# xipengwang/AprilSAM

Hardware: NVIDIA H100
Metric: Gauss-Newton solves/sec (batch + incremental) on M3500 & 100k-pose graph (higher is better)
Workload: dtype f64

## Files before the change

aprilsam_b200/csrc/asam_cuda.cu:

```cuda

#include <cuda_runtime.h>

#include <cmath>
#include <cstdarg>
#include <cstdint>
#include <cstdio>
#include <cstdlib>
#include <cstring>
#include <ctime>

#include "asam_cuda.h"

#define ASAM_EXPORT extern "C" __attribute__((visibility("default")))

static thread_local char g_err[512] = "";

static int set_err(const char *fmt, ...)
{
    va_list ap;
    va_start(ap, fmt);
    vsnprintf(g_err, sizeof(g_err), fmt, ap);
    va_end(ap);
    return 1;
}
// ... 457 lines not shown
        return set_err("no CUDA device");
    int dev = 0;
    const char *e = getenv("ASAM_DEVICE");
    if (!e)
        e = getenv("LOCAL_RANK");
    if (e)
        dev = atoi(e) % n;
    CK(cudaSetDevice(dev));
    asam_dev *d = new asam_dev();
    d->device = dev;
    cudaDeviceProp prop;
    CK(cudaGetDeviceProperties(&prop, dev));
    d->n_sm = prop.multiProcessorCount;
    CK(cudaStreamCreateWithFlags(&d->stream, cudaStreamNonBlocking));
    d->pin_cap = 8u << 20;
    CK(cudaMallocHost((void **) &d->pin, d->pin_cap));
    CK(cudaMalloc((void **) &d->dstage, d->pin_cap));
    d->items = (BatchItem *) malloc(ASAM_TABLE_BYTES);
    CK(cudaEventCreateWithFlags(&d->up_ev, cudaEventDisableTiming));
    d->pin_down_cap = 8u << 20;
    CK(cudaMallocHost((void **) &d->pin_down, d->pin_down_cap));
    for (int i = 0; i < 6; i++)
        CK(cudaEventCreate(&d->ev[i]));
    if (buf_reserve(d, d->ctrl, 8 * sizeof(int), false, true))
        return 1;

    int max_optin = 0;
    CK(cudaDeviceGetAttribute(&max_optin, cudaDevAttrMaxSharedMemoryPerBlockOptin, dev));
    const int want = 200 * 1024;
    if (want > max_optin - 1024)
        return set_err("k_factor needs %d KB of shared memory per block, the device offers %d KB", want / 1024,
                       (max_optin - 1024) / 1024);
    d->fac_smem = want;
    CK(cudaFuncSetAttribute(k_factor, cudaFuncAttributeMaxDynamicSharedMemorySize, d->fac_smem));
    int occ = 0;
    CK(cudaOccupancyMaxActiveBlocksPerMultiprocessor(&occ, k_factor, d->fac_threads, d->fac_smem));
    if (occ < 1)
        return set_err("k_factor does not fit on an SM");
    d->fac_grid = occ * d->n_sm;

    d->leaf_smem = ASAM_LEAF_WARPS * ASAM_LEAF_STRIDE * (int) sizeof(double);
    CK(cudaFuncSetAttribute(k_factor_leaf, cudaFuncAttributeMaxDynamicSharedMemorySize, d->leaf_smem));
    CK(cudaOccupancyMaxActiveBlocksPerMultiprocessor(&occ, k_factor_leaf, 32 * ASAM_LEAF_WARPS, d->leaf_smem));
    if (occ < 1)
        return set_err("k_factor_leaf does not fit on an SM");
    d->leaf_grid = occ * d->n_sm;

    d->bsl_smem = ASAM_BSL_WARPS * ASAM_BSL_STRIDE * (int) sizeof(double);
    CK(cudaFuncSetAttribute(k_backsolve_leaf, cudaFuncAttributeMaxDynamicSharedMemorySize, d->bsl_smem));
    CK(cudaOccupancyMaxActiveBlocksPerMultiprocessor(&occ, k_backsolve_leaf, 32 * ASAM_BSL_WARPS, d->bsl_smem));
    if (occ < 1)
        return set_err("k_backsolve_leaf does not fit on an SM");
    d->bsl_grid = occ * d->n_sm;

    if (getenv("ASAM_BS_THREADS"))
        d->bs_threads = atoi(getenv("ASAM_BS_THREADS")) >= 256 ? 256 : 128;
    d->bs_smem = 100 * 1024;
    CK(cudaFuncSetAttribute(k_backsolve, cudaFuncAttributeMaxDynamicSharedMemorySize, d->bs_smem));
    CK(cudaOccupancyMaxActiveBlocksPerMultiprocessor(&occ, k_backsolve, d->bs_threads, d->bs_smem));
    if (occ < 1)
        return set_err("k_backsolve does not fit on an SM");
    d->bs_grid = occ * d->n_sm;
    CK(cudaFuncSetAttribute(k_step, cudaFuncAttributeMaxDynamicSharedMemorySize, d->fac_smem));
    if (getenv("ASAM_SOLO_PB") && atoi(getenv("ASAM_SOLO_PB")) >= 12)
        d->solo_pb = atoi(getenv("ASAM_SOLO_PB")) / 12 * 12;
    if (getenv("ASAM_PB_SMEM") && atoi(getenv("ASAM_PB_SMEM")) >= 3)
        d->pb_smem = atoi(getenv("ASAM_PB_SMEM")) / 3 * 3;
    if (getenv("ASAM_SMEM_MMA"))
        d->smem_mma = atoi(getenv("ASAM_SMEM_MMA"));
    if (getenv("ASAM_DIAG_MMA")) {
        const int v = atoi(getenv("ASAM_DIAG_MMA")) != 0;
        CK(cudaMemcpyToSymbol(g_diag_mma, &v, sizeof(int)));
    }
    if (getenv("ASAM_DMAP_AHEAD")) {
        const int v = atoi(getenv("ASAM_DMAP_AHEAD")) != 0;
        CK(cudaMemcpyToSymbol(g_dmap_ahead, &v, sizeof(int)));
    }
    if (getenv("ASAM_PF_GROUPS")) {
        const int v = atoi(getenv("ASAM_PF_GROUPS")) != 0;
        CK(cudaMemcpyToSymbol(g_pf_groups, &v, sizeof(int)));
    }
    if (getenv("ASAM_KEEP"))
        d->keep_off = atoi(getenv("ASAM_KEEP")) == 0;
    if (getenv("ASAM_TILE_MODE"))
        d->tile_mode = atoi(getenv("ASAM_TILE_MODE"));
    if (getenv("ASAM_SMALL_STEP"))
        d->small_ok = atoi(getenv("ASAM_SMALL_STEP")) != 0;
    memset(d->pin_down, 0, 64);
    *out = d;
    return 0;
}

ASAM_EXPORT void asam_dev_destroy(asam_dev_t *d)
{
    if (!d)
        return;
    cudaSetDevice(d->device);
    cudaStreamSynchronize(d->stream);
    Buf *all[] = { &d->f_type, &d->f_a, &d->f_b, &d->f_z, &d->f_W, &d->f_slot, &d->lp, &d->st, &d->node2q, &d->q2node,
                   &d->Adiag, &d->Aoff, &d->Bq, &d->y, &d->x, &d->dinv, &d->sn, &d->ipool, &d->arena, &d->arrive,
                   &d->xdone, &d->xblk, &d->tbar, &d->tasks_full, &d->nwait_full, &d->btasks_full, &d->tasks_tmp, &d->nwait_tmp,
                   &d->btasks_tmp, &d->keep_tmp, &d->leaf_tasks, &d->top_tasks, &d->top_nwait, &d->ctrl, &d->partial, &d->patch_ids, &d->patch_desc, &d->pts, &d->flush, &d->trace_fac, &d->trace_bs, &d->ptrace };
    for (int i = 0; i < 2; i++)
        if (d->tev[i])
            cudaEventDestroy(d->tev[i]);
    for (Buf *b : all)
        if (b->p)
            cudaFree(b->p);
    if (d->pin)
        cudaFreeHost(d->pin);
    if (d->pin_down)
        cudaFreeHost(d->pin_down);
    if (d->dstage)
        cudaFree(d->dstage);
    if (d->up_ev)
        cudaEventDestroy(d->up_ev);
    free(d->items);
    free(d->pend);
    free(d->sh_owner); free(d->sh_q0); free(d->sh_qn); free(d->sh_off); free(d->sh_cnt);
    for (int i = 0; i < 6; i++)
        if (d->ev[i])
            cudaEventDestroy(d->ev[i]);
    cudaStreamDestroy(d->stream);
    delete d;
}

ASAM_EXPORT int asam_reserve(asam_dev_t *d, int n_nodes, int n_factors, int n_slots, int n_sn, int64_t ipool_ints,
                             int64_t arena_doubles)
{
    CK(cudaSetDevice(d->device));
    size_t N = (size_t) (n_nodes > 0 ? n_nodes : 0), Fn = (size_t) (n_factors > 0 ? n_factors : 0);
    size_t S = (size_t) (n_slots > 0 ? n_slots : 0), SN = (size_t) (n_sn > 0 ? n_sn : 0);
    int rc = 0;
    rc |= buf_reserve(d, d->f_type, Fn * sizeof(int), true, false);
    rc |= buf_reserve(d, d->f_a, Fn * sizeof(int), true, false);
    rc |= buf_reserve(d, d->f_b, Fn * sizeof(int), true, false);
    rc |= buf_reserve(d, d->f_slot, Fn * sizeof(int), true, false);
    rc |= buf_reserve(d, d->f_z, Fn * 3 * sizeof(double), true, false);
    rc |= buf_reserve(d, d->f_W, Fn * 9 * sizeof(double), true, false);
    rc |= buf_reserve(d, d->lp, N * 3 * sizeof(double), true, false);
    rc |= buf_reserve(d, d->st, N * 3 * sizeof(double), true, false);
    rc |= buf_reserve(d, d->node2q, N * sizeof(int), true, false);
    rc |= buf_reserve(d, d->q2node, N * sizeof(int), true, false);
    rc |= buf_reserve(d, d->Adiag, N * 9 * sizeof(double), true, true);
    rc |= buf_reserve(d, d->Bq, N * 3 * sizeof(double), true, true);
    rc |= buf_reserve(d, d->y, N * 3 * sizeof(double), true, true);
    rc |= buf_reserve(d, d->x, N * 3 * sizeof(double), true, true);
    rc |= buf_reserve(d, d->dinv, N * 3 * sizeof(double), true, true);
    rc |= buf_reserve(d, d->Aoff, S * 9 * sizeof(double), true, true);
    rc |= buf_reserve(d, d->sn, SN * sizeof(asam_sn_desc_t), true, false);
    rc |= buf_reserve(d, d->arrive, SN * sizeof(int), true, true);
    rc |= buf_reserve(d, d->xdone, SN * sizeof(int), true, true);
    rc |= buf_reserve(d, d->xblk, SN * sizeof(int), true, true);
    rc |= buf_reserve(d, d->tbar, 2 * SN * sizeof(int), true, true);
    rc |= buf_reserve(d, d->ipool, (size_t) ipool_ints * sizeof(int), true, false);
    rc |= buf_reserve(d, d->arena, (size_t) arena_doubles * sizeof(double), true, false);
    return rc;
}

ASAM_EXPORT int asam_upload_factors(asam_dev_t *d, int first, int count, const int32_t *type, const int32_t *na,
                                    const int32_t *nb, const double *z3, const double *W9)
{
    if (count <= 0)
        return 0;
    size_t need = (size_t) first + count;
    if (need * sizeof(int) > d->f_type.cap)
        return set_err("asam_upload_factors: capacity (call asam_reserve)");
    int rc = 0;
    rc |= upload(d, (int *) d->f_type.p + first, type, count * sizeof(int));
    rc |= upload(d, (int *) d->f_a.p + first, na, count * sizeof(int));
    rc |= upload(d, (int *) d->f_b.p + first, nb, count * sizeof(int));
    rc |= upload(d, (double *) d->f_z.p + 3 * (size_t) first, z3, count * 3 * sizeof(double));
    rc |= upload(d, (double *) d->f_W.p + 9 * (size_t) first, W9, count * 9 * sizeof(double));
    return rc;
}

ASAM_EXPORT int asam_upload_points(asam_dev_t *d, int which, int first, int count, const double *p3)
{
    if (count <= 0)
        return 0;
    Buf &b = which == 0 ? d->lp : d->st;
    if (((size_t) first + count) * 3 * sizeof(double) > b.cap)
        return set_err("asam_upload_points: capacity");
    return upload(d, (double *) b.p + 3 * (size_t) first, p3, (size_t) count * 3 * sizeof(double));
}

ASAM_EXPORT int asam_copy_points(asam_dev_t *d, int from, int to, int first, int count)
{
    if (count <= 0 || from == to)
        return 0;
    CK(cudaSetDevice(d->device));
    Buf &src = from == 0 ? d->lp : d->st, &dst = to == 0 ? d->lp : d->st;
    const size_t off = (size_t) first * 3 * sizeof(double), bytes = (size_t) count * 3 * sizeof(double);
    if (off + bytes > src.cap || off + bytes > dst.cap)
        return set_err("asam_copy_points: capacity");
    if (flush_uploads(d))
        return 1;
    CK(cudaMemcpyAsync((char *) dst.p + off, (const char *) src.p + off, bytes, cudaMemcpyDeviceToDevice, d->stream));
    return 0;
}

ASAM_EXPORT int asam_upload_node2q(asam_dev_t *d, int first, int count, const int32_t *node2q)
{
    if (count <= 0)
        return 0;
    if (((size_t) first + count) * sizeof(int) > d->node2q.cap)
        return set_err("asam_upload_node2q: capacity");
    return upload(d, (int *) d->node2q.p + first, node2q, (size_t) count * sizeof(int));
}

ASAM_EXPORT int asam_upload_q2node(asam_dev_t *d, int first, int count, const int32_t *q2node)
{
    if (count <= 0)
        return 0;
    if (((size_t) first + count) * sizeof(int) > d->q2node.cap)
        return set_err("asam_upload_q2node: capacity");
    return upload(d, (int *) d->q2node.p + first, q2node, (size_t) count * sizeof(int));
}

ASAM_EXPORT int asam_upload_fslot(asam_dev_t *d, int first, int count, const int32_t *fslot)
{
    if (count <= 0)
        return 0;
    if (((size_t) first + count) * sizeof(int) > d->f_slot.cap)
        return set_err("asam_upload_fslot: capacity");
    return upload(d, (int *) d->f_slot.p + first, fslot, (size_t) count * sizeof(int));
}

ASAM_EXPORT int asam_upload_ipool(asam_dev_t *d, int64_t first, int64_t count, const int32_t *data)
{
    if (count <= 0)
        return 0;
    if ((size_t) (first + count) * sizeof(int) > d->ipool.cap)
        return set_err("asam_upload_ipool: capacity");
    return upload(d, (int *) d->ipool.p + first, data, (size_t) count * sizeof(int));
}

ASAM_EXPORT int asam_upload_desc(asam_dev_t *d, int n, const int32_t *sn_ids, const asam_sn_desc_t *desc)
{
    if (n <= 0)
        return 0;
    CK(cudaSetDevice(d->device));
    if (n <= 256) {
        for (int i = 0; i < n; i++)
            if (upload(d, (asam_sn_desc_t *) d->sn.p + sn_ids[i], &desc[i], sizeof(asam_sn_desc_t)))
                return 1;
        return 0;
    }
    if (buf_reserve(d, d->patch_ids, (size_t) n * sizeof(int), false, false))
        return 1;
    if (buf_reserve(d, d->patch_desc, (size_t) n * sizeof(asam_sn_desc_t), false, false))
        return 1;
    if (upload(d, d->patch_ids.p, sn_ids, (size_t) n * sizeof(int)))
        return 1;
    if (upload(d, d->patch_desc.p, desc, (size_t) n * sizeof(asam_sn_desc_t)))
        return 1;
    if (flush_uploads(d))
        return 1;
    k_apply_desc<<<(n + 127) / 128, 128, 0, d->stream>>>((asam_sn_desc_t *) d->sn.p, (const int *) d->patch_ids.p,
                                                         (const asam_sn_desc_t *) d->patch_desc.p, n);
    d->n_launch++;
    CK(cudaGetLastError());
    return 0;
}

ASAM_EXPORT int asam_hessian_reset(asam_dev_t *d, int n_nodes, int n_slots, int n_lambda, double lambda)
{
    CK(cudaSetDevice(d->device));
    size_t total = 9 * (size_t) n_nodes + 9 * (size_t) n_slots + 3 * (size_t) n_nodes;
    if (total == 0)
        return 0;
    if (flush_uploads(d))
        return 1;
    k_hessian_reset<<<(unsigned) ((total + 255) / 256), 256, 0, d->stream>>>(
        (double *) d->Adiag.p, (double *) d->Aoff.p, (double *) d->Bq.p, n_nodes, n_slots, n_lambda, lambda);
    d->n_launch++;
    CK(cudaGetLastError());
    return 0;
}

ASAM_EXPORT int asam_hessian_clear_range(asam_dev_t *d, int q_first, int q_count, int slot_first, int slot_count)
{
    CK(cudaSetDevice(d->device));
    int rc = 0;
    if (q_count > 0) {
        rc |= queue_fill(d, (double *) d->Adiag.p + 9 * (size_t) q_first, 0, (size_t) q_count * 9 * sizeof(double));
        rc |= queue_fill(d, (double *) d->Bq.p + 3 * (size_t) q_first, 0, (size_t) q_count * 3 * sizeof(double));
    }
    if (slot_count > 0)
        rc |= queue_fill(d, (double *) d->Aoff.p + 9 * (size_t) slot_first, 0, (size_t) slot_count * 9 * sizeof(double));
    return rc;
}

ASAM_EXPORT int asam_linearize(asam_dev_t *d, int f_first, int f_count, const double *pts6)
{
    if (f_count <= 0)
        return 0;
    CK(cudaSetDevice(d->device));
    LinArgs a;
    a.f_type = (const int *) d->f_type.p;
    a.f_a = (const int *) d->f_a.p;
    a.f_b = (const int *) d->f_b.p;
    a.f_slot = (const int *) d->f_slot.p;
    a.f_z = (const double *) d->f_z.p;
    a.f_W = (const double *) d->f_W.p;
    a.lp = (const double *) d->lp.p;
    a.st = (const double *) d->st.p;
// ... 759 lines not shown
```

aprilsam_b200/csrc/asam_kernels.cuh:

```cuda
#pragma once

#include <cuda_runtime.h>

#include <cstdint>

#include "asam_cuda.h"

#define ASAM_TR_FLAG (1 << 30)
#define ASAM_MAX_CACHED_CHILDREN 24

__device__ __forceinline__ double d_mod2pi(double v)
{
    const double twopi = 6.2831853071795862319959;
    const double pi = 3.141592653589793238462643383279502884196;
    double w = v + pi;
    return (w - twopi * floor(w / twopi)) - pi;
}

__device__ __forceinline__ void d_atb(const double *A, const double *B, double *C)
{
#pragma unroll
    for (int i = 0; i < 3; i++)
#pragma unroll
        for (int j = 0; j < 3; j++) {
// ... 554 lines not shown
                    for (int u = 0; u < 8; u++)
                        Li[lane + 32 * u + pp * ASAM_LDI] = vi[h][u];
                }
            }
        }
    }
    const int g = lane >> 2, t = lane & 3;
    const int r0 = warp * 8 * MT;
    const int nnt = (ncol + 7) >> 3;
    const int rowmax = rb0 + min(r0 + 8 * MT, nrow) - 1;
    const int nneed = (r0 < nrow && rowmax >= cb0) ? min(nnt, ((rowmax - cb0) >> 3) + 1) : 0;
    double acc[MT][8][2];
#pragma unroll
    for (int mt = 0; mt < MT; mt++)
#pragma unroll
        for (int q = 0; q < 8; q++)
#pragma unroll
            for (int e = 0; e < 2; e++) {
                const int ii = r0 + 8 * mt + g, jj = 8 * q + 2 * t + e;
                const bool ok = q < nneed && ii < nrow && jj < ncol && rb0 + ii >= cb0 + jj;
                acc[mt][q][e] = ok ? __ldcg(&F[(rb0 + ii) + (size_t) (cb0 + jj) * ld]) : 0.0;
            }
    if (bulk) {
        mbar_wait(bar, parity);
        parity ^= 1u;
    }
    __syncthreads();
    if (nneed > 0) {
        const double *ai = Li + shi + r0 + g + (size_t) t * ASAM_LDI;
        const double *bj_ = Lj + shj + g + (size_t) t * ASAM_LDJ;
#pragma unroll 2
        for (int kk = 0; kk < pb4; kk += 4) {
            double av[MT];
#pragma unroll
            for (int mt = 0; mt < MT; mt++)
                av[mt] = -ai[8 * mt + (size_t) kk * ASAM_LDI];
#pragma unroll
            for (int q = 0; q < 8; q++) {
                if (q < nneed) {
                    const double bv = bj_[8 * q + (size_t) kk * ASAM_LDJ];
#pragma unroll
                    for (int mt = 0; mt < MT; mt++)
                        dmma_8x8x4(acc[mt][q][0], acc[mt][q][1], av[mt], bv);
                }
            }
        }
#pragma unroll
        for (int mt = 0; mt < MT; mt++)
#pragma unroll
            for (int q = 0; q < 8; q++)
#pragma unroll
                for (int e = 0; e < 2; e++) {
                    const int ii = r0 + 8 * mt + g, jj = 8 * q + 2 * t + e;
                    if (q < nneed && ii < nrow && jj < ncol && rb0 + ii >= cb0 + jj) {
                        F[(rb0 + ii) + (size_t) (cb0 + jj) * ld] = acc[mt][q][e];
                        if (Dout)
                            Dout[ii + jj * ASAM_TPB] = acc[mt][q][e];
                    }
                }
    }
}

#define ASAM_LDW 52
#define ASAM_WS_DOUBLES(m) (2 * (size_t) ((m) + 2) * ASAM_LDW)

template <int MT>
__device__ __noinline__ void tile_rm(double *F, const int ld, const double *Wk, const int pb4, const int cb0, const int ncol,
                                     const int rb0, const int nrow, const int out_mode, double *Out, double *Li, double *Lj,
                                     unsigned long long *bar, unsigned &parity)
{
    const int tid = threadIdx.x;
    const int lane = tid & 31, warp = tid >> 5;
    const bool same = rb0 == cb0 && nrow >= ncol;
    __syncthreads();
    if (warp == 0) {
        asm volatile("fence.proxy.async;" ::: "memory");
        if (lane == 0) {
            const unsigned bi = (unsigned) nrow * ASAM_LDW * 8u, bj = same ? 0u : (unsigned) ncol * ASAM_LDW * 8u;
            mbar_expect_tx(bar, bi + bj);
            bulk_g2s(Li, Wk + (size_t) rb0 * ASAM_LDW, bi, bar);
            if (!same)
                bulk_g2s(Lj, Wk + (size_t) cb0 * ASAM_LDW, bj, bar);
        }
    }
    const double *Ljs = same ? Li : Lj;
    const int g = lane >> 2, t = lane & 3;
    const int r0 = warp * 8 * MT;
    const int nnt = (ncol + 7) >> 3;
    const int rowmax = rb0 + min(r0 + 8 * MT, nrow) - 1;
    const int nneed = (r0 < nrow && rowmax >= cb0) ? min(nnt, ((rowmax - cb0) >> 3) + 1) : 0;
    double acc[MT][8][2];
#pragma unroll
    for (int mt = 0; mt < MT; mt++)
#pragma unroll
        for (int q = 0; q < 8; q++)
#pragma unroll
            for (int e = 0; e < 2; e++) {
                const int ii = r0 + 8 * mt + g, jj = 8 * q + 2 * t + e;
                const bool ok = q < nneed && ii < nrow && jj < ncol && rb0 + ii >= cb0 + jj;
                acc[mt][q][e] = ok ? __ldcg(&F[(rb0 + ii) + (size_t) (cb0 + jj) * ld]) : 0.0;
            }
    mbar_wait(bar, parity);
    parity ^= 1u;
    if (nneed > 0) {
        const double *ai = Li + (size_t) (r0 + g) * ASAM_LDW + t;
        const double *bj_ = Ljs + (size_t) g * ASAM_LDW + t;
#pragma unroll 2
        for (int kk = 0; kk < pb4; kk += 4) {
            double av[MT];
#pragma unroll
            for (int mt = 0; mt < MT; mt++)
                av[mt] = -ai[(size_t) (8 * mt) * ASAM_LDW + kk];
#pragma unroll
            for (int q = 0; q < 8; q++) {
                if (q < nneed) {
                    const double bv = bj_[(size_t) (8 * q) * ASAM_LDW + kk];
#pragma unroll
                    for (int mt = 0; mt < MT; mt++)
                        dmma_8x8x4(acc[mt][q][0], acc[mt][q][1], av[mt], bv);
                }
            }
        }
    }
    if (out_mode == 2)
        __syncthreads();
    if (nneed > 0) {
#pragma unroll
        for (int mt = 0; mt < MT; mt++)
#pragma unroll
            for (int q = 0; q < 8; q++)
#pragma unroll
                for (int e = 0; e < 2; e++) {
                    const int ii = r0 + 8 * mt + g, jj = 8 * q + 2 * t + e;
                    if (q < nneed && ii < nrow && jj < ncol && rb0 + ii >= cb0 + jj) {
                        if (out_mode == 0)
                            F[(rb0 + ii) + (size_t) (cb0 + jj) * ld] = acc[mt][q][e];
                        else if (out_mode == 1)
                            Out[ii + jj * ASAM_TPB] = acc[mt][q][e];
                        else
                            Out[ii + jj * ASAM_TROWS] = acc[mt][q][e];
                    }
                }
    }
}

struct TeamCtx {
    int *tbar_s;
    int G, w, phase;
    long long spin_limit;
    int *err;
    int sn;
};

__device__ __forceinline__ bool team_barrier(TeamCtx &tc, int *s_flag)
{
    __syncthreads();
    if (threadIdx.x == 0) {
        red_release_add(tc.tbar_s, 1);
        const int target = (++tc.phase) * tc.G;
        SpinClock spins;
        int ok = 1;
        while (ld_volatile(tc.tbar_s) < target) {
            __nanosleep(20);
            if (spin_over(spins, tc.spin_limit) || ld_volatile(tc.err) < 0) {
                atomicCAS(tc.err, 0, -(1 + tc.sn));
                ok = 0;
                break;
            }
        }
        ld_acquire(tc.tbar_s);
        *s_flag = ok;
    } else {
        tc.phase++;
    }
    __syncthreads();
    return *s_flag != 0;
}

__device__ __forceinline__ void team_leave(TeamCtx &tc)
{
    if (threadIdx.x == 0) {
        const int v = atomicAdd(tc.tbar_s, 1);
        if (v == tc.phase * tc.G + tc.G - 1)
            atomicExch(tc.tbar_s, 0);
    }
}

__device__ __forceinline__ bool team_owns(int col, int w, int G) { return ((col >> 2) % G) == w; }

__device__ __forceinline__ void diag_factor(double *D, int pb, double *rdv, int sn_id, int *err)
{
    const int tid = threadIdx.x;
    constexpr int LDD = ASAM_TPB;
    for (int c0 = 0; c0 < pb; c0 += 3) {
        if (c0 > 0 && tid < 3 * (pb - c0)) {
            const int i = c0 + tid / 3, j = c0 + tid % 3;
            if (i >= j) {
                double acc0 = D[i + j * LDD], acc1 = 0.0;
                int p = 0;
                for (; p + 1 < c0; p += 2) {
                    acc0 -= D[i + p * LDD] * D[j + p * LDD];
                    acc1 -= D[i + (p + 1) * LDD] * D[j + (p + 1) * LDD];
                }
                if (p < c0)
                    acc0 -= D[i + p * LDD] * D[j + p * LDD];
                D[i + j * LDD] = acc0 + acc1;
            }
        }
        __syncthreads();
        double *p0 = D + c0 * LDD, *p1 = p0 + LDD, *p2 = p1 + LDD;
        const double a00 = p0[c0], a10 = p0[c0 + 1], a20 = p0[c0 + 2];
        const double a11 = p1[c0 + 1], a21 = p1[c0 + 2], a22 = p2[c0 + 2];
        const double r0 = d_rsqrt(a00);
        const double l10 = a10 * r0, l20 = a20 * r0;
        const double d1 = a11 - l10 * l10;
        const double r1 = d_rsqrt(d1);
        const double l21 = (a21 - l20 * l10) * r1;
        const double d2 = a22 - l20 * l20 - l21 * l21;
        const double r2 = d_rsqrt(d2);
        if (tid == 0 && !(a00 > 0.0 && d1 > 0.0 && d2 > 0.0))
            atomicCAS(err, 0, 1 + sn_id);
        const int i = c0 + 3 + tid;
        if (i < pb) {
            const double x0 = p0[i] * r0;
            const double x1 = (p1[i] - x0 * l10) * r1;
            const double x2 = (p2[i] - x0 * l20 - x1 * l21) * r2;
            p0[i] = x0;
            p1[i] = x1;
            p2[i] = x2;
        }
        __syncthreads();
        if (tid == 0) {
            p0[c0] = a00 * r0; p0[c0 + 1] = l10; p0[c0 + 2] = l20;
            p1[c0 + 1] = d1 * r1; p1[c0 + 2] = l21;
            p2[c0 + 2] = d2 * r2;
            rdv[c0] = r0; rdv[c0 + 1] = r1; rdv[c0 + 2] = r2;
        }
    }
    __syncthreads();
}

__device__ __forceinline__ void diag_factor_rl(double *D, int pb, double *rdv, int sn_id, int *err)
{
    constexpr int LDD = ASAM_TPB;
    constexpr int SUB = 256;
    if (threadIdx.x < SUB) {
        for (int k1 = 0; k1 < pb; k1 += ASAM_PB) {
            const int pbb = min(ASAM_PB, pb - k1);
            panel_factor(D + (size_t) k1 * LDD, LDD, k1, pbb, pb - 1, sn_id, err, rdv, SUB);
            if (k1 + pbb < pb) {
                if (g_diag_mma)
                    trailing_update_mma(D, LDD, D + (size_t) k1 * LDD, LDD, pbb, k1 + pbb, pb, pb - 1, SUB / 32);
                else
                    trailing_update<1, 4>(D, LDD, D + (size_t) k1 * LDD, LDD, pbb, k1 + pbb, pb, pb - 1, SUB / 32);
                bar_sub(SUB);
            }
        }
    }
    __syncthreads();
}

__device__ __forceinline__ void trsm_row_block(double *Li, const double *D, const double *rdv, const int b0, const int nb,
                                               double *Frow, int ld, double *Wrow)
{
    const int tid = threadIdx.x;
    constexpr int LDD = ASAM_TPB;
    double r[12];
#pragma unroll
    for (int q = 0; q < 12; q++)
        r[q] = (q < nb) ? Li[tid + (b0 + q) * ASAM_TROWS] : 0.0;
    for (int p = 0; p < b0; p++) {
        const double xp = Li[tid + p * ASAM_TROWS];
        const double2 *Dp = reinterpret_cast<const double2 *>(D + p * LDD + b0);
#pragma unroll
        for (int q2 = 0; q2 < 6; q2++) {
            const double2 v = Dp[q2];
            r[2 * q2] -= xp * v.x;
            r[2 * q2 + 1] -= xp * v.y;
        }
    }
#pragma unroll
    for (int q = 0; q < 12; q++) {
        if (q < nb) {
            r[q] *= rdv[b0 + q];
#pragma unroll
            for (int q2 = q + 1; q2 < 12; q2++)
                r[q2] -= r[q] * D[(b0 + q2) + (b0 + q) * LDD];
        }
    }
#pragma unroll
    for (int q = 0; q < 12; q++)
        if (q < nb) {
            Li[tid + (b0 + q) * ASAM_TROWS] = r[q];
            Frow[(size_t) (b0 + q) * ld] = r[q];
            if (Wrow)
                Wrow[b0 + q] = r[q];
        }
}

__device__ __forceinline__ void trsm_row(double *Li, const double *D, const double *rdv, int pb, double *Frow, int ld,
                                         double *Wrow = nullptr)
{
    for (int b0 = 0; b0 < pb; b0 += 12)
        trsm_row_block(Li, D, rdv, b0, min(12, pb - b0), Frow, ld, Wrow);
    if (Wrow)
        for (int q = pb; q < ((pb + 3) & ~3); q++)
            Wrow[q] = 0.0;
}

__device__ bool team_front(const FacArgs &a, const asam_sn_desc_t &d, int s, int nw, int w, int G, double *sm,
                           int *s_flag, unsigned long long *trow, unsigned long long *mbar, unsigned &mb_parity)
{
    const int tid = threadIdx.x, nt = blockDim.x;
    const int lane = tid & 31, warp = tid >> 5, nwarps = nt >> 5;
    const int m = 3 * d.mb, c = 3 * d.cb, ld = ASAM_LD(m);
    const int *seg = a.ipool + d.seg;
    const int *children = seg + 2 * d.mb;
    const int *a_slot = children + d.ch_cnt;
    const int *a_rb = a_slot + d.a_cnt;
    const int *a_cb = a_rb + d.a_cnt;
    double *F = a.arena + d.f_off;
    int *err = a.ctrl + 1;
    TeamCtx tc;
    tc.tbar_s = a.tbar + 2 * (size_t) s;
    tc.G = G;
    tc.w = w;
    tc.phase = 0;
    tc.spin_limit = a.spin_limit;
    tc.err = err;
    tc.sn = s;

    for (int j = warp; j < m; j += nwarps) {
        if (!team_owns(j, w, G))
            continue;
        for (int i = j + lane; i <= m; i += 32)
            F[i + (size_t) j * ld] = 0.0;
    }
    __syncthreads();
    for (int e = tid; e < d.cb * 9; e += nt) {
        int k = e / 9, p = (e % 9) / 3, q = e % 3;
        if (p >= q && team_owns(3 * k + q, w, G))
            F[(3 * k + p) + (size_t) (3 * k + q) * ld] = a.Adiag[9 * (size_t) a.q2node[d.first + k] + q * 3 + p];
    }
    for (int e = tid; e < c; e += nt)
        if (team_owns(e, w, G))
            F[m + (size_t) e * ld] = a.Bq[3 * (size_t) a.q2node[d.first + e / 3] + e % 3];
    for (int e = tid; e < d.a_cnt * 9; e += nt) {
        int i = e / 9, p = (e % 9) / 3, q = e % 3;
        const int col = 3 * a_cb[i] + q;
        if (!team_owns(col, w, G))
            continue;
        const int rbf = a_rb[i];
        const int rb = rbf & ~ASAM_TR_FLAG;
        const int si = (rbf & ASAM_TR_FLAG) ? (p * 3 + q) : (q * 3 + p);
        F[(3 * rb + p) + (size_t) col * ld] = a.Aoff[9 * (size_t) a_slot[i] + si];
    }
    if (nw > 0 && tid == 0) {
        SpinClock spins;
        int ok = 1;
        while (ld_volatile(&a.arrive[s]) < nw) {
            __nanosleep(20);
            if (spin_over(spins, a.spin_limit) || ld_volatile(err) < 0) {
                atomicCAS(err, 0, -(1 + s));
                ok = 0;
                break;
            }
        }
        __threadfence();
        *s_flag = ok;
    } else if (tid == 0) {
        *s_flag = 1;
    }
    __syncthreads();
    if (!*s_flag)
        return false;
    if (trow && tid == 0)
        trow[1] = trow[2] = d_now();

    int *dmap = (int *) sm;
    for (int ci = 0; ci < d.ch_cnt; ++ci) {
        const asam_sn_desc_t cd = a.sn[children[ci]];
        const int cm = 3 * cd.mb, cc = 3 * cd.cb, cr = cm - cc, cld = ASAM_LD(cm);
        const double *CF = a.arena + cd.f_off;
        const int *crel = a.ipool + cd.seg + cd.mb;
        __syncthreads();
        for (int i = tid; i <= cr; i += nt)
            dmap[i] = (i < cr) ? 3 * crel[(cc + i) / 3] + (cc + i) % 3 : m;
        __syncthreads();
        for (int j = warp; j < cr; j += nwarps) {
            const int dj = dmap[j];
            if (!team_owns(dj, w, G))
                continue;
            const double *ccol = CF + (size_t) (cc + j) * cld + cc;
            double *fcol = F + (size_t) dj * ld;
            for (int i0 = j + lane; i0 <= cr; i0 += 256) {
                double v[8], dv[8];
                int di[8];
#pragma unroll
                for (int u = 0; u < 8; u++) {
                    const bool ok = i0 + 32 * u <= cr;
                    v[u] = ok ? __ldcg(ccol + i0 + 32 * u) : 0.0;
                    di[u] = ok ? dmap[i0 + 32 * u] : -1;
                }
#pragma unroll
                for (int u = 0; u < 8; u++)
                    dv[u] = di[u] >= 0 ? __ldcg(fcol + di[u]) : 0.0;
#pragma unroll
                for (int u = 0; u < 8; u++)
                    if (di[u] >= 0)
                        fcol[di[u]] = dv[u] + v[u];
            }
        }
    }
    if (!team_barrier(tc, s_flag))
        return false;
    if (w == 0 && nw > 0 && tid == 0)
        a.arrive[s] = 0;
    unsigned long long t_panel = 0, t_mark = 0;
    if (trow && tid == 0)
        trow[3] = d_now();

    double *D = sm;
    double *rdv = D + ASAM_TPB * ASAM_TPB;
    double *Li = rdv + ASAM_TPB;
    double *Lj = Li + ASAM_LDI * ASAM_TPB;
    const bool v3 = a.tile_mode == 3;
    double *Wbase = F + (size_t) ld * m;
    auto Wbuf = [&](int panel_index) { return Wbase + (size_t) (panel_index & 1) * (m + 2) * ASAM_LDW; };
    double *Lj3 = Li + ASAM_TROWS * ASAM_LDW;
    double *dinv = a.dinv + 3 * (size_t) d.first;
    int *crew_bar = a.tbar + 2 * (size_t) s + 1;

    auto tile = [&](int k0, int pb, int cb0, int ncol, int rb0, int nrow, double *Dout) {
        if (v3) {
            const double *Wk = Wbuf(k0 / ASAM_TPB);
            const int pb4 = (pb + 3) & ~3;
            if (Dout)
                tile_rm<1>(F, ld, Wk, pb4, cb0, ncol, rb0, nrow, 1, Dout, Li, Lj3, mbar, mb_parity);
            else if (nrow <= 128)
                tile_rm<2>(F, ld, Wk, pb4, cb0, ncol, rb0, nrow, 0, nullptr, Li, Lj3, mbar, mb_parity);
            else
                tile_rm<4>(F, ld, Wk, pb4, cb0, ncol, rb0, nrow, 0, nullptr, Li, Lj3, mbar, mb_parity);
            return;
        }
        if (a.tile_mode != 0) {
            const int bulk = a.tile_mode == 2;
            if (nrow <= 64)
                tile_mma<1>(F, ld, m, k0, pb, cb0, ncol, rb0, nrow, Dout, Li, Lj, mbar, mb_parity, bulk);
            else if (nrow <= 128)
                tile_mma<2>(F, ld, m, k0, pb, cb0, ncol, rb0, nrow, Dout, Li, Lj, mbar, mb_parity, bulk);
            else
                tile_mma<4>(F, ld, m, k0, pb, cb0, ncol, rb0, nrow, Dout, Li, Lj, mbar, mb_parity, bulk);
            return;
        }
        __syncthreads();
        for (int p = warp; p < pb; p += 2 * nwarps) {
            double vj[2][2], vi[2][8];
#pragma unroll
            for (int h = 0; h < 2; h++) {
                const int pp = p + h * nwarps;
                const double *src = F + (size_t) (k0 + min(pp, pb - 1)) * ld;
#pragma unroll
                for (int u = 0; u < 2; u++)
                    vj[h][u] = (pp < pb && lane + 32 * u < ncol) ? __ldcg(src + cb0 + lane + 32 * u) : 0.0;
#pragma unroll
                for (int u = 0; u < 8; u++)
                    vi[h][u] = (pp < pb && lane + 32 * u < nrow) ? __ldcg(src + rb0 + lane + 32 * u) : 0.0;
            }
#pragma unroll
            for (int h = 0; h < 2; h++) {
                const int pp = p + h * nwarps;
                if (pp < pb) {
#pragma unroll
                    for (int u = 0; u < 2; u++)
                        if (lane + 32 * u < ncol)
                            Lj[lane + 32 * u + pp * ASAM_TCOLS] = vj[h][u];
#pragma unroll
                    for (int u = 0; u < 8; u++)
                        if (lane + 32 * u < nrow)
                            Li[lane + 32 * u + pp * ASAM_TROWS] = vi[h][u];
                }
            }
        }
        __syncthreads();
        const int tj = 8 * warp;
        if (tj < ncol) {
            for (int ib = 0; ib < nrow; ib += 128) {
                double acc[4][8], cv[4][8];
                int ir[4], jc[8];
#pragma unroll
                for (int q = 0; q < 8; q++)
                    jc[q] = min(tj + q, ncol - 1);
#pragma unroll
                for (int r = 0; r < 4; r++) {
                    ir[r] = min(ib + lane + 32 * r, nrow - 1);
#pragma unroll
                    for (int q = 0; q < 8; q++) {
                        acc[r][q] = 0.0;
                        const int ii = ib + lane + 32 * r, jj = tj + q;
                        const bool ok = ii < nrow && jj < ncol && rb0 + ii >= cb0 + jj;
                        cv[r][q] = ok ? __ldcg(&F[(rb0 + ii) + (size_t) (cb0 + jj) * ld]) : 0.0;
                    }
                }
#pragma unroll 2
                for (int p = 0; p < pb; p++) {
                    double bq[8], av[4];
#pragma unroll
                    for (int q = 0; q < 8; q++)
                        bq[q] = Lj[jc[q] + p * ASAM_TCOLS];
#pragma unroll
                    for (int r = 0; r < 4; r++)
                        av[r] = Li[ir[r] + p * ASAM_TROWS];
#pragma unroll
                    for (int r = 0; r < 4; r++)
#pragma unroll
                        for (int q = 0; q < 8; q++)
                            acc[r][q] += av[r] * bq[q];
                }
#pragma unroll
                for (int r = 0; r < 4; r++)
#pragma unroll
                    for (int q = 0; q < 8; q++) {
                        const int ii = ib + lane + 32 * r, jj = tj + q;
                        const int i = rb0 + ii, j = cb0 + jj;
                        if (ii < nrow && jj < ncol && i >= j) {
                            const double v = cv[r][q] - acc[r][q];
                            F[i + (size_t) j * ld] = v;
                            if (Dout)
                                Dout[ii + jj * ASAM_TPB] = v;
                        }
                    }
            }
        }
    };
    auto panel = [&](int k0, int pb, int rb0) {
        __syncthreads();
        for (int e = tid; e < ASAM_TPB * ASAM_TPB; e += nt) {
            const int i = e % ASAM_TPB, j = e / ASAM_TPB;
            D[e] = (i >= j && i < pb && j < pb) ? __ldcg(&F[(k0 + i) + (size_t) (k0 + j) * ld]) : 0.0;
        }
        const int i = rb0 + tid;
        const bool row = rb0 >= 0 && i >= k0 + pb && i <= m;
        if (row)
            for (int j = 0; j < pb; j++)
                Li[tid + j * ASAM_TROWS] = __ldcg(&F[i + (size_t) (k0 + j) * ld]);
        __syncthreads();
        if (v3)
            diag_factor_rl(D, pb, rdv, s, err);
        else
            diag_factor(D, pb, rdv, s, err);
        if (row)
            trsm_row(Li, D, rdv, pb, F + i + (size_t) k0 * ld, ld, v3 ? Wbuf(0) + (size_t) i * ASAM_LDW : nullptr);
    };
    auto writeback = [&](int k0, int pb) {
        for (int e = tid; e < pb * pb; e += nt) {
            const int i = e % pb, j = e / pb;
            if (i >= j)
                F[(k0 + i) + (size_t) (k0 + j) * ld] = D[i + j * ASAM_TPB];
        }
        for (int e = tid; e < pb; e += nt)
            dinv[k0 + e] = rdv[e];
    };

    auto diag_publish = [&](int k0, int pb, int seq) {
        __syncthreads();
        if (v3) {
            constexpr int LDD = ASAM_TPB;
            constexpr int SUB = 256;
            int stage = 0;
            for (int k1 = 0; k1 < pb; k1 += ASAM_PB) {
                const int pbb = min(ASAM_PB, pb - k1);
                panel_factor(D + (size_t) k1 * LDD, LDD, k1, pbb, pb - 1, s, err, rdv, SUB);
                ++stage;
                for (int e = tid; e < pbb * pb; e += SUB) {
                    const int j = k1 + e / pb, i = e % pb;
                    if (i >= j)
                        F[(k0 + i) + (size_t) (k0 + j) * ld] = D[i + j * LDD];
                }
                for (int e = tid; e < pbb; e += SUB)
                    dinv[k0 + k1 + e] = rdv[k1 + e];
                bar_sub(SUB);
                if (tid == 0)
                    st_release(crew_bar, 8 * seq + stage);
                if (k1 + pbb < pb) {
                    if (g_diag_mma)
                        trailing_update_mma(D, LDD, D + (size_t) k1 * LDD, LDD, pbb, k1 + pbb, pb, pb - 1, SUB / 32);
                    else
                        trailing_update<1, 4>(D, LDD, D + (size_t) k1 * LDD, LDD, pbb, k1 + pbb, pb, pb - 1, SUB / 32);
                    bar_sub(SUB);
                }
            }
            __syncthreads();
            return;
        }
        diag_factor(D, pb, rdv, s, err);
        writeback(k0, pb);
        __syncthreads();
        if (tid == 0) {
            __threadfence();
            atomicExch(crew_bar, seq);
        }
    };
    auto rows_solve_staged = [&](int k0, int pb, int rb0, int seq, double *Wnext) {
        constexpr int LDD = ASAM_TPB;
        if (tid == 0)
            *s_flag = 1;
        __syncthreads();
        const int i = rb0 + tid;
        const bool row = tid < ASAM_CROWS && i <= m;
        int stage = 0;
        for (int b0 = 0; b0 < pb; b0 += ASAM_PB, ++stage) {
            const int nb = min(ASAM_PB, pb - b0);
            if (warp >= 4) {
                if (tid == 128 && *s_flag) {
                    SpinClock spins;
                    while (ld_volatile(crew_bar) < 8 * seq + stage + 1) {
                        __nanosleep(20);
                        if (spin_over(spins, a.spin_limit) || ld_volatile(err) < 0) {
                            atomicCAS(err, 0, -(1 + s));
                            *s_flag = 0;
                            break;
                        }
                    }
                    ld_acquire(crew_bar);
                }
                asm volatile("bar.sync 2, 128;" ::: "memory");
                if (*s_flag) {
                    for (int e = tid - 128; e < nb * ASAM_TPB; e += 128) {
                        const int j = b0 + e / ASAM_TPB, ii = e % ASAM_TPB;
                        D[ii + j * LDD] = (ii >= j && ii < pb) ? __ldcg(&F[(k0 + ii) + (size_t) (k0 + j) * ld]) : 0.0;
                    }
                    if (tid - 128 < nb)
                        rdv[b0 + tid - 128] = __ldcg(&dinv[k0 + b0 + tid - 128]);
                }
                __threadfence_block();
                asm volatile("bar.arrive %0, 256;" ::"r"(3 + stage) : "memory");
            } else {
                asm volatile("bar.sync %0, 256;" ::"r"(3 + stage) : "memory");
                if (row && *s_flag)
                    trsm_row_block(Li, D, rdv, b0, nb, F + i + (size_t) k0 * ld, ld, Wnext + (size_t) i * ASAM_LDW);
            }
        }
        if (row && *s_flag)
            for (int q = pb; q < ((pb + 3) & ~3); q++)
                Wnext[(size_t) i * ASAM_LDW + q] = 0.0;
        __syncthreads();
        return *s_flag != 0;
    };
    auto rows_solve = [&](int k0, int pb, int rb0, int seq, double *Wnext) {
        __syncthreads();
        const int i = rb0 + tid;
        const bool row = tid < ASAM_CROWS && i <= m;
        if (row && !Wnext)
            for (int j = 0; j < pb; j++)
                Li[tid + j * ASAM_TROWS] = __ldcg(&F[i + (size_t) (k0 + j) * ld]);
        if (tid == 0) {
            SpinClock spins;
            int ok = 1;
            while (ld_volatile(crew_bar) < seq) {
                __nanosleep(20);
                if (spin_over(spins, a.spin_limit) || ld_volatile(err) < 0) {
                    atomicCAS(err, 0, -(1 + s));
                    ok = 0;
                    break;
                }
            }
            __threadfence();
            *s_flag = ok;
        }
        __syncthreads();
        if (!*s_flag)
            return false;
        for (int e = tid; e < ASAM_TPB * ASAM_TPB; e += nt) {
            const int ii = e % ASAM_TPB, j = e / ASAM_TPB;
            D[e] = (ii >= j && ii < pb && j < pb) ? __ldcg(&F[(k0 + ii) + (size_t) (k0 + j) * ld]) : 0.0;
        }
        for (int e = tid; e < ASAM_TPB; e += nt)
            rdv[e] = e < pb ? __ldcg(&dinv[k0 + e]) : 0.0;
        __syncthreads();
        if (row)
            trsm_row(Li, D, rdv, pb, F + i + (size_t) k0 * ld, ld, Wnext ? Wnext + (size_t) i * ASAM_LDW : nullptr);
        return true;
    };

    {
        const int pb = min(ASAM_TPB, c);
        if (trow && tid == 0)
            t_mark = d_now();
        const int nchunk = (m + 1 + ASAM_TROWS - 1) / ASAM_TROWS;
        bool first = true;
        for (int ch = w; ch < nchunk || first; ch += G) {
            panel(0, pb, ch < nchunk ? ch * ASAM_TROWS : -1);
            first = false;
        }
        if (!team_barrier(tc, s_flag))
            return false;
        if (trow && tid == 0)
            t_panel += d_now() - t_mark;
        if (w == 0)
            writeback(0, pb);
    }
    int seq = 0;
    const bool pt_on = a.ptrace && s == a.ptrace_sn && w < 8 && tid == 0;
    for (int k0 = 0; k0 < c; k0 += ASAM_TPB) {
        unsigned long long *pt = (pt_on && k0 / ASAM_TPB < a.ptrace_panels) ? a.ptrace + ((size_t) (k0 / ASAM_TPB) * 8 + w) * 8 : nullptr;
        if (pt) {
            pt[0] = d_now();
            pt[1] = pt[2] = pt[3] = pt[0];
            pt[5] = (unsigned long long) m;
            pt[6] = (unsigned long long) G;
        }
        const int pb = min(ASAM_TPB, c - k0);
        const int kn0 = k0 + pb;
        const bool has_next = kn0 < c;
        const int pbn = has_next ? min(ASAM_TPB, c - kn0) : 0;
        const int ncrew = has_next ? 1 + (m - (kn0 + pbn) + 1 + ASAM_CROWS - 1) / ASAM_CROWS : 0;
        ++seq;
        if (w < ncrew) {
            if (trow && tid == 0)
                t_mark = d_now();
            if (w == 0) {
                __syncthreads();
                for (int e = tid; e < ASAM_TPB * ASAM_TPB; e += nt)
                    D[e] = 0.0;
                tile(k0, pb, kn0, pbn, kn0, pbn, D);
                if (pt)
                    pt[1] = d_now();
                diag_publish(kn0, pbn, seq);
                if (pt)
                    pt[2] = d_now();
            }
            if (v3) {
                for (int it = (w == 0 ? G : w); it < ncrew; it += G) {
                    const int rb0 = kn0 + pbn + (it - 1) * ASAM_CROWS;
                    tile_rm<2>(F, ld, Wbuf(k0 / ASAM_TPB), (pb + 3) & ~3, kn0, pbn, rb0, min(ASAM_CROWS, m - rb0 + 1), 2, Li, Li,
                               Lj3, mbar, mb_parity);
                    if (pt && w > 0 && it == w)
                        pt[1] = d_now();
                    if (!rows_solve_staged(kn0, pbn, rb0, seq, Wbuf(kn0 / ASAM_TPB)))
                        return false;
                }
            } else {
                for (int it = (w == 0 ? G : w); it < ncrew; it += G) {
                    const int rb0 = kn0 + pbn + (it - 1) * ASAM_CROWS;
                    tile(k0, pb, kn0, pbn, rb0, min(ASAM_CROWS, m - rb0 + 1), nullptr);
                }
                if (pt && w > 0)
                    pt[1] = d_now();
                for (int it = (w == 0 ? G : w); it < ncrew; it += G) {
                    const int rb0 = kn0 + pbn + (it - 1) * ASAM_CROWS;
                    if (!rows_solve(kn0, pbn, rb0, seq, nullptr))
                        return false;
                }
            }
            if (pt && w > 0)
                pt[2] = d_now();
            if (trow && tid == 0)
                t_panel += d_now() - t_mark;
        }

        const int j0 = kn0 + pbn;
        const int nfree = (G - ncrew >= 2) ? G - ncrew : G, wfree = (G - ncrew >= 2) ? w - ncrew : w;
        int n256 = 0;
        for (int cb0 = j0; cb0 < m; cb0 += ASAM_TCOLS)
            n256 += (m - cb0 + 1 + 255) / 256;
        const int TR = (n256 < 2 * nfree) ? 128 : 256;
        if (wfree >= 0) {
            int u = 0;
            for (int cb0 = j0; cb0 < m; cb0 += ASAM_TCOLS)
                for (int rb0 = cb0; rb0 <= m; rb0 += TR, ++u)
                    if (u % nfree == wfree)
                        tile(k0, pb, cb0, min(ASAM_TCOLS, m - cb0), rb0, min(TR, m - rb0 + 1), nullptr);
        }
        if (pt)
            pt[3] = d_now();
        if (!team_barrier(tc, s_flag))
            return false;
        if (pt) {
            pt[4] = d_now();
            pt[7] = (unsigned long long) ncrew;
        }
    }
    if (w == 0 && tid == 0)
        atomicExch(crew_bar, 0);

    if (trow && tid == 0) {
        trow[4] = d_now();
        trow[7] = (unsigned long long) (unsigned) m | (t_panel << 32);
    }
    if (w == 0) {
        for (int e = tid; e < c; e += nt)
            a.y[3 * (size_t) d.first + e] = __ldcg(&F[m + (size_t) e * ld]);
        __syncthreads();
        if (tid == 0 && d.parent >= 0) {
            __threadfence();
            atomicAdd(&a.arrive[d.parent], 1);
        }
    }
    team_leave(tc);
    __syncthreads();
    return true;
}

__device__ __forceinline__ void ticket_release(int *ticket, int *done)
{
    __syncthreads();
    if (threadIdx.x == 0) {
        __threadfence();
        if (atomicAdd(done, 1) == (int) gridDim.x - 1) {
            atomicExch(ticket, 0);
            atomicExch(done, 0);
        }
    }
}

__device__ bool cta_front(const FacArgs &a, const int t, const int s, const int nw, const asam_sn_desc_t &d, double *sm,
                          asam_sn_desc_t *s_cd, int *s_abort, unsigned long long tr0, const int keepw = 0)
{
    const int tid = threadIdx.x, nt = blockDim.x;
    const int lane = tid & 31, warp = tid >> 5, nwarps = nt >> 5;
    int *err = a.ctrl + 1;
    unsigned long long tr1 = 0, tr2 = 0, tr3 = 0, tr4 = 0, accA = 0, accB = 0;
    const int m = 3 * d.mb, c = 3 * d.cb, ld = ASAM_LD(m);
    const int *seg = a.ipool + d.seg;
    const int *children = seg + 2 * d.mb;
    const int *a_slot = children + d.ch_cnt;
    const int *a_rb = a_slot + d.a_cnt;
    const int *a_cb = a_rb + d.a_cnt;
    double *Fg = a.arena + d.f_off;
    const long long fsz = (long long) ld * m;
    const bool use_sm = fsz + (ld + 1) / 2 + 2 <= (long long) a.smem_doubles;
    double *F = use_sm ? sm : Fg;
    int *dmap = (int *) (sm + (use_sm ? fsz : 0));
    double *Pbuf = sm + (ld + 1) / 2 + 1;
    double *dinv = a.dinv + 3 * (size_t) d.first;

    if (use_sm) {
        for (int i = tid; i < (int) fsz; i += nt)
            F[i] = 0.0;
    } else {
        for (int j = warp; j < m; j += nwarps)
            for (int i = j + lane; i <= m; i += 32)
                F[i + (size_t) j * ld] = 0.0;
    }
    for (int e = tid; e < d.ch_cnt && e < ASAM_MAX_CACHED_CHILDREN; e += nt)
        s_cd[e] = a.sn[children[e]];
    __syncthreads();
    __shared__ int s_doff[ASAM_MAX_CACHED_CHILDREN + 1];
    bool dmap_ahead = false;
    if (use_sm && g_dmap_ahead && d.ch_cnt > 0 && d.ch_cnt <= ASAM_MAX_CACHED_CHILDREN) {
        if (tid == 0) {
            int o = 0;
            for (int e = 0; e < d.ch_cnt; e++) {
                s_doff[e] = o;
                o += 3 * (s_cd[e].mb - s_cd[e].cb) + 1;
            }
            s_doff[d.ch_cnt] = o;
        }
        __syncthreads();
        dmap_ahead = (long long) s_doff[d.ch_cnt] <= 2 * ((long long) a.smem_doubles - fsz) - 2;
        if (dmap_ahead)
            for (int ci = 0; ci < d.ch_cnt; ++ci) {
                const int cc = 3 * s_cd[ci].cb, cr = 3 * s_cd[ci].mb - cc;
                const int *crel = a.ipool + s_cd[ci].seg + s_cd[ci].mb;
                int *dm = dmap + s_doff[ci];
                for (int i = tid; i <= cr; i += nt)
                    dm[i] = (i < cr) ? 3 * crel[(cc + i) / 3] + (cc + i) % 3 : m;
            }
    }
    for (int e = tid; e < d.cb * 9; e += nt) {
        int k = e / 9, p = (e % 9) / 3, q = e % 3;
        if (p >= q)
            F[(3 * k + p) + (size_t) (3 * k + q) * ld] =
                a.Adiag[9 * (size_t) a.q2node[d.first + k] + q * 3 + p];
    }
    for (int e = tid; e < c; e += nt)
        F[m + (size_t) e * ld] = a.Bq[3 * (size_t) a.q2node[d.first + e / 3] + e % 3];
    for (int e = tid; e < d.a_cnt * 9; e += nt) {
        int i = e / 9, p = (e % 9) / 3, q = e % 3;
        const int rbf = a_rb[i];
        const int rb = rbf & ~ASAM_TR_FLAG;
        const int si = (rbf & ASAM_TR_FLAG) ? (p * 3 + q) : (q * 3 + p);
        F[(3 * rb + p) + (size_t) (3 * a_cb[i] + q) * ld] = a.Aoff[9 * (size_t) a_slot[i] + si];
    }
    if (a.trace && tid == 0)
        tr1 = d_now();

    if (nw > 0 && tid == 0) {
        SpinClock spins;
        while (ld_volatile(&a.arrive[s]) < nw) {
            __nanosleep(32);
            if (spin_over(spins, a.spin_limit) || ld_volatile(err) < 0) {
                atomicCAS(err, 0, -(1 + s));
                *s_abort = 1;
                break;
            }
        }
        a.arrive[s] = 0;
        __threadfence();
    }
    __syncthreads();
    if (*s_abort)
        return false;
    if (a.trace && tid == 0)
        tr2 = d_now();

    for (int ci = 0; ci < d.ch_cnt; ++ci) {
        const asam_sn_desc_t cd = ci < ASAM_MAX_CACHED_CHILDREN ? s_cd[ci] : a.sn[children[ci]];
        const int cm = 3 * cd.mb, cc = 3 * cd.cb, cr = cm - cc, cld = ASAM_LD(cm);
        const double *CF = a.arena + cd.f_off;
        const int *crel = a.ipool + cd.seg + cd.mb;
        if (dmap_ahead) {
            dmap = (int *) (sm + fsz) + s_doff[ci];
        } else {
            for (int i = tid; i <= cr; i += nt)
                dmap[i] = (i < cr) ? 3 * crel[(cc + i) / 3] + (cc + i) % 3 : m;
            __syncthreads();
        }
        if (use_sm && cr <= 159) {
            for (int j0 = warp; j0 < cr; j0 += 4 * nwarps) {
                double v[4][5];
#pragma unroll
                for (int q = 0; q < 4; q++) {
                    const int j = j0 + q * nwarps;
                    const double *ccol = CF + (size_t) (cc + min(j, cr - 1)) * cld + cc;
#pragma unroll
                    for (int u = 0; u < 5; u++) {
                        const int i = j + lane + 32 * u;
                        v[q][u] = (j < cr && i <= cr) ? __ldcg(ccol + i) : 0.0;
                    }
                }
#pragma unroll
                for (int q = 0; q < 4; q++) {
                    const int j = j0 + q * nwarps;
                    if (j < cr) {
                        double *fcol = F + (size_t) dmap[j] * ld;
#pragma unroll
// ... 960 lines not shown
```

Measured before the change: 128.8.

## Let leader block start next panel diag early via split barrier and ready counter

Splits the team barrier into separate arrive and wait phases and adds a per-supernode ready counter. In tile mode 3, worker 0 arrives at the barrier but skips the wait, then waits only until the specific blocks its next diagonal tile depends on (first crew row solve and first trailing tile) are done. This lets the next panel's diagonal factorization overlap the rest of the trailing update. The cost is an extra sync counter per supernode and subtler ordering logic, which could introduce races or deadlocks.

```diff
diff --git a/aprilsam_b200/csrc/asam_cuda.cu b/aprilsam_b200/csrc/asam_cuda.cu
--- a/aprilsam_b200/csrc/asam_cuda.cu
+++ b/aprilsam_b200/csrc/asam_cuda.cu
@@ -633,7 +633,7 @@
     rc |= buf_reserve(d, d->arrive, SN * sizeof(int), true, true);
     rc |= buf_reserve(d, d->xdone, SN * sizeof(int), true, true);
     rc |= buf_reserve(d, d->xblk, SN * sizeof(int), true, true);
-    rc |= buf_reserve(d, d->tbar, 2 * SN * sizeof(int), true, true);
+    rc |= buf_reserve(d, d->tbar, 3 * SN * sizeof(int), true, true);
     rc |= buf_reserve(d, d->ipool, (size_t) ipool_ints * sizeof(int), true, false);
     rc |= buf_reserve(d, d->arena, (size_t) arena_doubles * sizeof(double), true, false);
     return rc;
diff --git a/aprilsam_b200/csrc/asam_kernels.cuh b/aprilsam_b200/csrc/asam_kernels.cuh
--- a/aprilsam_b200/csrc/asam_kernels.cuh
+++ b/aprilsam_b200/csrc/asam_kernels.cuh
@@ -730,12 +730,18 @@
     int sn;
 };
 
-__device__ __forceinline__ bool team_barrier(TeamCtx &tc, int *s_flag)
+__device__ __forceinline__ void team_arrive(TeamCtx &tc)
 {
     __syncthreads();
+    if (threadIdx.x == 0)
+        red_release_add(tc.tbar_s, 1);
+    tc.phase++;
+}
+
+__device__ __forceinline__ bool team_wait(TeamCtx &tc, int *s_flag)
+{
     if (threadIdx.x == 0) {
-        red_release_add(tc.tbar_s, 1);
-        const int target = (++tc.phase) * tc.G;
+        const int target = tc.phase * tc.G;
         SpinClock spins;
         int ok = 1;
         while (ld_volatile(tc.tbar_s) < target) {
@@ -748,11 +754,15 @@
         }
         ld_acquire(tc.tbar_s);
         *s_flag = ok;
-    } else {
-        tc.phase++;
     }
     __syncthreads();
     return *s_flag != 0;
+}
+
+__device__ __forceinline__ bool team_barrier(TeamCtx &tc, int *s_flag)
+{
+    team_arrive(tc);
+    return team_wait(tc, s_flag);
 }
 
 __device__ __forceinline__ void team_leave(TeamCtx &tc)
@@ -900,7 +910,7 @@
     double *F = a.arena + d.f_off;
     int *err = a.ctrl + 1;
     TeamCtx tc;
-    tc.tbar_s = a.tbar + 2 * (size_t) s;
+    tc.tbar_s = a.tbar + 3 * (size_t) s;
     tc.G = G;
     tc.w = w;
     tc.phase = 0;
@@ -1007,7 +1017,8 @@
     auto Wbuf = [&](int panel_index) { return Wbase + (size_t) (panel_index & 1) * (m + 2) * ASAM_LDW; };
     double *Lj3 = Li + ASAM_TROWS * ASAM_LDW;
     double *dinv = a.dinv + 3 * (size_t) d.first;
-    int *crew_bar = a.tbar + 2 * (size_t) s + 1;
+    int *crew_bar = tc.tbar_s + 1;
+    int *blk_ready = tc.tbar_s + 2;
 
     auto tile = [&](int k0, int pb, int cb0, int ncol, int rb0, int nrow, double *Dout) {
         if (v3) {
@@ -1278,6 +1289,30 @@
         if (w == 0)
             writeback(0, pb);
     }
+    bool pend = false;
+    auto wait_ready = [&](int v) {
+        if (tid == 0) {
+            SpinClock spins;
+            int ok = 1;
+            while (ld_volatile(blk_ready) < v) {
+                __nanosleep(20);
+                if (spin_over(spins, a.spin_limit) || ld_volatile(err) < 0) {
+                    atomicCAS(err, 0, -(1 + s));
+                    ok = 0;
+                    break;
+                }
+            }
+            ld_acquire(blk_ready);
+            *s_flag = ok;
+        }
+        __syncthreads();
+        return *s_flag != 0;
+    };
+    auto raise_ready = [&]() {
+        __syncthreads();
+        if (tid == 0)
+            red_release_add(blk_ready, 1);
+    };
     int seq = 0;
     const bool pt_on = a.ptrace && s == a.ptrace_sn && w < 8 && tid == 0;
     for (int k0 = 0; k0 < c; k0 += ASAM_TPB) {
@@ -1298,6 +1333,8 @@
             if (trow && tid == 0)
                 t_mark = d_now();
             if (w == 0) {
+                if (pend && !wait_ready(2 * (seq - 1)))
+                    return false;
                 __syncthreads();
                 for (int e = tid; e < ASAM_TPB * ASAM_TPB; e += nt)
                     D[e] = 0.0;
@@ -1308,6 +1345,11 @@
                 if (pt)
                     pt[2] = d_now();
             }
+            if (pend) {
+                if (!team_wait(tc, s_flag))
+                    return false;
+                pend = false;
+            }
             if (v3) {
                 for (int it = (w == 0 ? G : w); it < ncrew; it += G) {
                     const int rb0 = kn0 + pbn + (it - 1) * ASAM_CROWS;
@@ -1317,6 +1359,8 @@
                         pt[1] = d_now();
                     if (!rows_solve_staged(kn0, pbn, rb0, seq, Wbuf(kn0 / ASAM_TPB)))
                         return false;
+                    if (it == 1)
+                        raise_ready();
                 }
             } else {
                 for (int it = (w == 0 ? G : w); it < ncrew; it += G) {
@@ -1335,6 +1379,11 @@
                 pt[2] = d_now();
             if (trow && tid == 0)
                 t_panel += d_now() - t_mark;
+        }
+        if (pend) {
+            if (!team_wait(tc, s_flag))
+                return false;
+            pend = false;
         }
 
         const int j0 = kn0 + pbn;
@@ -1347,20 +1396,29 @@
             int u = 0;
             for (int cb0 = j0; cb0 < m; cb0 += ASAM_TCOLS)
                 for (int rb0 = cb0; rb0 <= m; rb0 += TR, ++u)
-                    if (u % nfree == wfree)
+                    if (u % nfree == wfree) {
                         tile(k0, pb, cb0, min(ASAM_TCOLS, m - cb0), rb0, min(TR, m - rb0 + 1), nullptr);
+                        if (v3 && u == 0)
+                            raise_ready();
+                    }
         }
         if (pt)
             pt[3] = d_now();
-        if (!team_barrier(tc, s_flag))
+        if (v3 && w == 0 && has_next) {
+            team_arrive(tc);
+            pend = true;
+        } else if (!team_barrier(tc, s_flag)) {
             return false;
+        }
         if (pt) {
             pt[4] = d_now();
             pt[7] = (unsigned long long) ncrew;
         }
     }
-    if (w == 0 && tid == 0)
+    if (w == 0 && tid == 0) {
         atomicExch(crew_bar, 0);
+        atomicExch(blk_ready, 0);
+    }
 
     if (trow && tid == 0) {
         trow[4] = d_now();
```

After: 131.2, median of 6. 1.02x the previous value.
